# 3SAILab/two_stage_object_detection

Hardware: AMD Instinct MI355X
Metric: images/sec Faster R-CNN ResNet-50 @800x1333 (higher is better)
Workload: dtype f32 storage/accumulate; conv products as bf16x3 (3 exact bf16 pieces per operand, 6 bf16 MFMAs per product) in 0 of 43 conv layers, as fp16x2 (2 fp16 pieces of 2^e x per operand, 3 fp16 MFMAs per product; e follows the tensor's abs-max per forward: range words) in 43, f32 MFMA in the rest; 1 GPU; Full Faster R-CNN resnet50 inference forward, batch=1 per GPU, 3x800x1333, 80+1 classes, 3000->300 proposals; global_batch=1, parallelism=dp1, hip_graph=True, autotuned_tiles=True, steps_in_flight=4, tiles_tuned_on=this rank

## Files before the change

### include/tsod.h

```cpp
#ifndef TSOD_H
#define TSOD_H

#include <stddef.h>
#include <stdint.h>

#ifdef __cplusplus
extern "C" {
#endif

#define TSOD_VERSION 242

typedef void *tsod_stream_t;

typedef enum tsod_status {
    TSOD_OK = 0,
    TSOD_ERR_INVALID_ARG = -1,
    TSOD_ERR_UNSUPPORTED = -2,
    TSOD_ERR_ALIGNMENT = -3,
    TSOD_ERR_WORKSPACE = -4,
    TSOD_ERR_LAUNCH = -5
} tsod_status;

const char *tsod_status_str(int status);
int tsod_version(void);
int tsod_device_cu_count(void);

enum { TSOD_ACT_NONE = 0, TSOD_ACT_PRELU = 1, TSOD_ACT_RELU6 = 2, TSOD_ACT_RELU = 3 };
enum { TSOD_TILE_AUTO = 0, TSOD_TILE_128x128 = 1, TSOD_TILE_128x64 = 2, TSOD_TILE_64x64 = 3, TSOD_TILE_64x128 = 4,
       TSOD_TILE_128x128_W8 = 5, TSOD_TILE_128x64_W8 = 6, TSOD_TILE_256x128_W8 = 7, TSOD_TILE_64x64_S1 = 8,
       TSOD_TILE_128x64_W8_S1 = 9, TSOD_TILE_64x64_S1_K64 = 10, TSOD_TILE_128x64_W8_S1_K64 = 11,
       TSOD_TILE_64x64_W1_S1 = 12, TSOD_TILE_128x64_W2_S1 = 13, TSOD_TILE_128x64_S1 = 14, TSOD_TILE_64x128_S1 = 15,
       TSOD_TILE_128x128_S1 = 16,
       TSOD_TILE_D128x128 = 17, TSOD_TILE_D64x128 = 18, TSOD_TILE_D256x128 = 19,
       TSOD_TILE_D64x128_S2 = 20 ,
       TSOD_TILE_D128x256 = 21 ,
       TSOD_TILE_D128x128_K32 = 22 ,
       TSOD_TILE_D192x128 = 23 ,
       TSOD_TILE_D64x128_K64 = 24 ,
       TSOD_TILE_COUNT = 25 };
enum { TSOD_PREC_F32 = 0, TSOD_PREC_BF16X3 = 1, TSOD_PREC_FP16X2 = 2 };
#define TSOD_MAX_SEGMENTS 16

typedef struct tsod_conv2d_desc {
    int32_t N, H, W;
    int32_t in_pitch;
    int32_t n_seg;
    int32_t seg_off[TSOD_MAX_SEGMENTS];
    int32_t seg_len[TSOD_MAX_SEGMENTS];
    int32_t Cout;
    int32_t out_pitch;
    int32_t out_off;
    int32_t KH, KW;
    int32_t stride;
    int32_t pad_h, pad_w;
    int32_t OH, OW;
    int32_t act;
    float slope;
    int32_t res_pitch;
    int32_t res_off;
    int32_t tile;
    int32_t split_k;
    int32_t precision;
    int32_t c2, in2_pitch, in2_off, stride2, H2, W2;
    int32_t a_scale_exp, w_scale_exp;
    int32_t *range_flag;
    const uint32_t *amax_in, *amax_in2;
    uint32_t *amax_out;
} tsod_conv2d_desc;

#define TSOD_AMAX_WORDS 64
#define TSOD_AMAX_STRIDE 64
#define TSOD_AMAX_BYTES (TSOD_AMAX_WORDS * TSOD_AMAX_STRIDE)
int tsod_amax_reset(uint32_t *words, int32_t n_tensors, tsod_stream_t stream);
int tsod_absmax_f32(const float *x, int64_t n, uint32_t *amax_out, tsod_stream_t stream);

int tsod_host_mapped_pointer(void *host, void **device);
int tsod_word_publish_i32(const int32_t *src_device, int32_t *dst_mapped, tsod_stream_t stream);

int tsod_pack_conv_weight_f32(const float *w_oihw, int32_t Cout, int32_t Cin_src, int32_t KH, int32_t KW_src,
                              int32_t Cin, int32_t KW, float *w_packed, tsod_stream_t stream);

size_t tsod_conv_weight_bf16x3_bytes(int32_t Cout, int32_t K);
int tsod_pack_conv_weight_bf16x3(const float *w_packed , int32_t Cout, int32_t K, void *w_bf16x3,
                                 tsod_stream_t stream);
size_t tsod_conv_weight_fp16x2_bytes(int32_t Cout, int32_t K);
int tsod_pack_conv_weight_fp16x2(const float *w_packed , int32_t Cout, int32_t K, int32_t w_scale_exp,
                                 void *w_fp16x2, tsod_stream_t stream);

size_t tsod_conv2d_workspace_bytes(const tsod_conv2d_desc *d);
int tsod_conv2d_resolve(const tsod_conv2d_desc *d, int32_t *tile, int32_t *split_k);

int tsod_conv2d_f32(const tsod_conv2d_desc *d, const float *in, const float *w_packed,
                    const float *scale , const float *shift ,
                    const float *residual , float *out,
                    void *workspace, size_t workspace_bytes, tsod_stream_t stream);

int tsod_conv2d_dual_f32(const tsod_conv2d_desc *d, const float *in, const float *in2, const float *w_packed,
                         const float *scale, const float *shift, const float *residual, float *out,
                         void *workspace, size_t workspace_bytes, tsod_stream_t stream);

typedef struct tsod_bottleneck_desc {
    int32_t N, H, W;
    int32_t Cin, in_pitch;
    int32_t Cmid;
    int32_t Cout, out_pitch;
    float slope;
    int32_t w_exp[3];
    int32_t a_scale_exp;
    int32_t projection;
    int32_t *range_flag;
    const uint32_t *amax_in;
    uint32_t *amax_out;
} tsod_bottleneck_desc;
size_t tsod_bottleneck_wstream_bytes(int32_t Cin, int32_t Cout);
size_t tsod_bottleneck_proj_wstream_bytes(int32_t Cin, int32_t Cout);
int tsod_bottleneck_fp16x2(const tsod_bottleneck_desc *d, const float *x, const void *wstream, const float *bn, float *out,
                           tsod_stream_t stream);

#define TSOD_STEM_NCHW 0
#define TSOD_STEM_NHWC4 1
typedef struct tsod_stem_desc {
    int32_t N, H, W;
    int32_t in_layout;
    int32_t out_pitch;
    float slope;
    int32_t w_exp;
    int32_t *range_flag;
    uint32_t *amax_out;
} tsod_stem_desc;
size_t tsod_stem_wfrag_bytes(void);
int tsod_stem_fp16x2(const tsod_stem_desc *d, const float *x, const void *wfrag, const float *bn, float *out, tsod_stream_t stream);

int tsod_linear_f32(const float *in, int32_t M, int32_t K, int32_t in_pitch, const float *w ,
                    const float *bias , int32_t N, float *out, int32_t out_pitch,
                    void *workspace, size_t workspace_bytes, tsod_stream_t stream);
size_t tsod_linear_workspace_bytes(int32_t M, int32_t K, int32_t N);

int tsod_maxpool3x3s2_f32(const float *in, int32_t N, int32_t H, int32_t W, int32_t C, int32_t in_pitch,
                          float *out, int32_t out_pitch, tsod_stream_t stream);

int tsod_dwconv3x3_f32(const float *in, int32_t N, int32_t H, int32_t W, int32_t C, int32_t in_pitch, int32_t in_off,
                       const float *w, const float *scale, const float *shift, int32_t stride, int32_t relu,
                       float *out, int32_t out_pitch, int32_t out_off, tsod_stream_t stream);

int tsod_dwconv3x3_amax_f32(const float *in, int32_t N, int32_t H, int32_t W, int32_t C, int32_t in_pitch, int32_t in_off,
                            const float *w, const float *scale, const float *shift, int32_t stride, int32_t relu,
                            float *out, int32_t out_pitch, int32_t out_off, uint32_t *amax_out, tsod_stream_t stream);

int tsod_gconv3x3_f32(const float *in, int32_t N, int32_t H, int32_t W, int32_t C, int32_t in_pitch, int32_t groups,
                      const float *w, const float *scale, const float *shift, int32_t stride, int32_t act, float slope,
                      float *out, int32_t out_pitch, tsod_stream_t stream);

int tsod_gconv3x3_amax_f32(const float *in, int32_t N, int32_t H, int32_t W, int32_t C, int32_t in_pitch, int32_t groups,
                           const float *w, const float *scale, const float *shift, int32_t stride, int32_t act, float slope,
                           float *out, int32_t out_pitch, uint32_t *amax_out, tsod_stream_t stream);

int tsod_gconv1x1_pair_f32(const float *in, int64_t pixels, int32_t G, int32_t in_pitch, const float *w,
                           const float *bias, float *out, int32_t out_pitch, tsod_stream_t stream);

int tsod_gconv1x1_pair_amax_f32(const float *in, int64_t pixels, int32_t G, int32_t in_pitch, const float *w,
                                const float *bias, float *out, int32_t out_pitch, uint32_t *amax_out, tsod_stream_t stream);

int tsod_nchw_to_nhwc_f32(const float *in, int32_t N, int32_t C, int32_t H, int32_t W,
                          float *out, int32_t out_pitch, int32_t C_pad, tsod_stream_t stream);
int tsod_nchw_to_nhwc_amax_f32(const float *in, int32_t N, int32_t C, int32_t H, int32_t W,
                               float *out, int32_t out_pitch, int32_t C_pad, uint32_t *amax_out, tsod_stream_t stream);
int tsod_nhwc_to_nchw_f32(const float *in, int32_t N, int32_t C, int32_t H, int32_t W, int32_t in_pitch,
                          int32_t in_off, float *out, tsod_stream_t stream);

int tsod_rpn_decode_f32(const float *locs, int32_t loc_pitch, const float *scores, int32_t score_pitch,
                        const float *anchor_base , int32_t A, int32_t B, int32_t Hf, int32_t Wf,
                        int32_t feat_stride, float clamp_x, float clamp_y, float min_size,
                        float *boxes, float *fg, float *keys, float *anchors_out, tsod_stream_t stream);
// ... 333 lines not shown
```

### two_stage_object_detection_amd/_ffi.py

```python
from __future__ import annotations

import ctypes
import os
from ctypes import POINTER, Structure, byref, c_char_p, c_double, c_float, c_int, c_int32, c_int64, c_size_t, c_void_p
from typing import NamedTuple

import torch

_PKG_DIR = os.path.dirname(os.path.abspath(__file__))
LIB_PATH = os.environ.get("TSOD_LIB") or os.path.join(_PKG_DIR, "libtsod.so")

TSOD_MAX_SEGMENTS = 16
AMAX_WORDS, AMAX_STRIDE = 64, 64
AMAX_BYTES = AMAX_WORDS * AMAX_STRIDE
ACT_NONE, ACT_PRELU, ACT_RELU6, ACT_RELU = 0, 1, 2, 3
PREC_F32, PREC_BF16X3, PREC_FP16X2 = 0, 1, 2
PREC_NAMES = {0: "f32", 1: "bf16x3", 2: "fp16x2"}
TILE_AUTO, TILE_128x128, TILE_128x64, TILE_64x64, TILE_64x128 = 0, 1, 2, 3, 4


class Tile(NamedTuple):
    name: str
    rows: int
    precisions: tuple
# ... 37 lines not shown
TILE_NAMES = {TILE_AUTO: "auto", **{t: row.name for t, row in TILES.items()}}
TILE_IDS = tile_ids(PREC_F32)
DMA_TILE_IDS = tuple(t for t, row in TILES.items() if row.dma)
BF16X3_TILE_IDS = tile_ids(PREC_BF16X3)
FP16X2_TILE_IDS = tile_ids(PREC_FP16X2)

class TsodError(RuntimeError):
    pass


class ConvDesc(Structure):
    _fields_ = [
        ("N", c_int32), ("H", c_int32), ("W", c_int32),
        ("in_pitch", c_int32), ("n_seg", c_int32),
        ("seg_off", c_int32 * TSOD_MAX_SEGMENTS), ("seg_len", c_int32 * TSOD_MAX_SEGMENTS),
        ("Cout", c_int32), ("out_pitch", c_int32), ("out_off", c_int32),
        ("KH", c_int32), ("KW", c_int32), ("stride", c_int32), ("pad_h", c_int32), ("pad_w", c_int32),
        ("OH", c_int32), ("OW", c_int32), ("act", c_int32), ("slope", c_float),
        ("res_pitch", c_int32), ("res_off", c_int32), ("tile", c_int32), ("split_k", c_int32), ("precision", c_int32),
        ("c2", c_int32), ("in2_pitch", c_int32), ("in2_off", c_int32), ("stride2", c_int32), ("H2", c_int32), ("W2", c_int32),
        ("a_scale_exp", c_int32), ("w_scale_exp", c_int32), ("range_flag", c_void_p),
        ("amax_in", c_void_p), ("amax_in2", c_void_p), ("amax_out", c_void_p),
    ]


class BottleneckDesc(Structure):
    _fields_ = [
        ("N", c_int32), ("H", c_int32), ("W", c_int32), ("Cin", c_int32), ("in_pitch", c_int32), ("Cmid", c_int32),
        ("Cout", c_int32), ("out_pitch", c_int32), ("slope", c_float), ("w_exp", c_int32 * 3), ("a_scale_exp", c_int32),
        ("projection", c_int32), ("range_flag", c_void_p), ("amax_in", c_void_p), ("amax_out", c_void_p),
    ]


class StemDesc(Structure):
    _fields_ = [
        ("N", c_int32), ("H", c_int32), ("W", c_int32), ("in_layout", c_int32), ("out_pitch", c_int32), ("slope", c_float),
        ("w_exp", c_int32), ("range_flag", c_void_p), ("amax_out", c_void_p),
    ]


STEM_NCHW, STEM_NHWC4 = 0, 1

AUG_MEAN_PARTS = 256
AUG_BRIGHTNESS, AUG_CONTRAST, AUG_SATURATION, AUG_HUE, AUG_CONTRAST_FIRST, AUG_PERMUTE = 1, 2, 4, 8, 16, 32


class Photometric(Structure):
    _fields_ = [("flags", c_int32), ("brightness", c_float), ("contrast", c_float), ("saturation", c_float),
                ("hue", c_float), ("white", c_float), ("perm", c_int32 * 3)]


PW_MAX_SEGMENTS = 16


class PwSegs(Structure):
    _fields_ = [("n_seg", c_int32), ("off", c_int32 * PW_MAX_SEGMENTS), ("len", c_int32 * PW_MAX_SEGMENTS),
                ("real", c_int32 * PW_MAX_SEGMENTS), ("want", c_int32 * PW_MAX_SEGMENTS)]


ADAMW_CHUNK, ADAMW_MAX_GROUPS = 2048, 32
BN_ROWS_PER_WORKGROUP = 128


class AdamWGroup(Structure):
    _fields_ = [("decay", c_float), ("one_minus_beta1", c_float), ("beta2", c_float), ("one_minus_beta2", c_float),
                ("step_size", c_float), ("bias2_sqrt", c_float), ("eps", c_float), ("reserved", c_float)]


class GradNormResult(Structure):
    _fields_ = [("sum_sq", c_double), ("norm", c_float), ("coef", c_float)]


_SIGNATURES = {
    "tsod_status_str": (c_char_p, [c_int]),
    "tsod_version": (c_int, []),
    "tsod_device_cu_count": (c_int, []),
    "tsod_pack_conv_weight_f32": (c_int, [c_void_p, c_int32, c_int32, c_int32, c_int32, c_int32, c_int32, c_void_p, c_void_p]),
    "tsod_conv_weight_bf16x3_bytes": (c_size_t, [c_int32, c_int32]),
    "tsod_pack_conv_weight_bf16x3": (c_int, [c_void_p, c_int32, c_int32, c_void_p, c_void_p]),
    "tsod_conv_weight_fp16x2_bytes": (c_size_t, [c_int32, c_int32]),
    "tsod_pack_conv_weight_fp16x2": (c_int, [c_void_p, c_int32, c_int32, c_int32, c_void_p, c_void_p]),
    "tsod_conv2d_workspace_bytes": (c_size_t, [POINTER(ConvDesc)]),
    "tsod_conv2d_resolve": (c_int, [POINTER(ConvDesc), POINTER(c_int32), POINTER(c_int32)]),
    "tsod_conv2d_f32": (c_int, [POINTER(ConvDesc), c_void_p, c_void_p, c_void_p, c_void_p, c_void_p, c_void_p,
                                c_void_p, c_size_t, c_void_p]),
    "tsod_conv2d_dual_f32": (c_int, [POINTER(ConvDesc), c_void_p, c_void_p, c_void_p, c_void_p, c_void_p, c_void_p, c_void_p,
                                     c_void_p, c_size_t, c_void_p]),
    "tsod_bottleneck_wstream_bytes": (c_size_t, [c_int32, c_int32]),
    "tsod_bottleneck_proj_wstream_bytes": (c_size_t, [c_int32, c_int32]),
    "tsod_bottleneck_fp16x2": (c_int, [POINTER(BottleneckDesc), c_void_p, c_void_p, c_void_p, c_void_p, c_void_p]),
    "tsod_stem_wfrag_bytes": (c_size_t, []),
    "tsod_stem_fp16x2": (c_int, [POINTER(StemDesc), c_void_p, c_void_p, c_void_p, c_void_p, c_void_p]),
    "tsod_linear_f32": (c_int, [c_void_p, c_int32, c_int32, c_int32, c_void_p, c_void_p, c_int32, c_void_p, c_int32,
                                c_void_p, c_size_t, c_void_p]),
    "tsod_linear_workspace_bytes": (c_size_t, [c_int32, c_int32, c_int32]),
    "tsod_maxpool3x3s2_f32": (c_int, [c_void_p, c_int32, c_int32, c_int32, c_int32, c_int32, c_void_p, c_int32, c_void_p]),
    "tsod_dwconv3x3_f32": (c_int, [c_void_p, c_int32, c_int32, c_int32, c_int32, c_int32, c_int32, c_void_p, c_void_p,
                                   c_void_p, c_int32, c_int32, c_void_p, c_int32, c_int32, c_void_p]),
    "tsod_dwconv3x3_amax_f32": (c_int, [c_void_p, c_int32, c_int32, c_int32, c_int32, c_int32, c_int32, c_void_p, c_void_p,
                                        c_void_p, c_int32, c_int32, c_void_p, c_int32, c_int32, c_void_p, c_void_p]),
    "tsod_gconv3x3_amax_f32": (c_int, [c_void_p, c_int32, c_int32, c_int32, c_int32, c_int32, c_int32, c_void_p, c_void_p, c_void_p,
                                       c_int32, c_int32, c_float, c_void_p, c_int32, c_void_p, c_void_p]),
    "tsod_gconv1x1_pair_amax_f32": (c_int, [c_void_p, c_int64, c_int32, c_int32, c_void_p, c_void_p, c_void_p, c_int32, c_void_p, c_void_p]),
    "tsod_nchw_to_nhwc_amax_f32": (c_int, [c_void_p, c_int32, c_int32, c_int32, c_int32, c_void_p, c_int32, c_int32, c_void_p, c_void_p]),
    "tsod_absmax_f32": (c_int, [c_void_p, c_int64, c_void_p, c_void_p]),
    "tsod_amax_reset": (c_int, [c_void_p, c_int32, c_void_p]),
    "tsod_host_mapped_pointer": (c_int, [c_void_p, c_void_p]),
    "tsod_word_publish_i32": (c_int, [c_void_p, c_void_p, c_void_p]),
    "tsod_gconv3x3_f32": (c_int, [c_void_p, c_int32, c_int32, c_int32, c_int32, c_int32, c_int32, c_void_p, c_void_p, c_void_p,
                                  c_int32, c_int32, c_float, c_void_p, c_int32, c_void_p]),
    "tsod_gconv1x1_pair_f32": (c_int, [c_void_p, c_int64, c_int32, c_int32, c_void_p, c_void_p, c_void_p, c_int32, c_void_p]),
    "tsod_nchw_to_nhwc_f32": (c_int, [c_void_p, c_int32, c_int32, c_int32, c_int32, c_void_p, c_int32, c_int32, c_void_p]),
    "tsod_nhwc_to_nchw_f32": (c_int, [c_void_p, c_int32, c_int32, c_int32, c_int32, c_int32, c_int32, c_void_p, c_void_p]),
    "tsod_rpn_decode_f32": (c_int, [c_void_p, c_int32, c_void_p, c_int32, c_void_p, c_int32, c_int32, c_int32, c_int32,
                                    c_int32, c_float, c_float, c_float, c_void_p, c_void_p, c_void_p, c_void_p, c_void_p]),
    "tsod_proposal_decode_f32": (c_int, [c_void_p, c_void_p, c_void_p, c_int64, c_float, c_float, c_float, c_void_p,
                                         c_void_p, c_void_p]),
    "tsod_enumerate_anchors_f32": (c_int, [c_void_p, c_int32, c_int32, c_int32, c_int32, c_void_p, c_void_p]),
    "tsod_loc2bbox_f32": (c_int, [c_void_p, c_void_p, c_int64, c_void_p, c_void_p]),
    "tsod_bbox2loc_f32": (c_int, [c_void_p, c_void_p, c_int64, c_void_p, c_void_p]),
    "tsod_sort_topk_desc_f32": (c_int, [c_void_p, c_void_p, c_int32, c_int32, c_int32, c_void_p, c_void_p, c_void_p,
                                        c_void_p, c_void_p]),
    "tsod_sort_topk_workspace_bytes": (c_size_t, [c_int32, c_int32, c_int32]),
    "tsod_sort_topk_desc_ws_f32": (c_int, [c_void_p, c_void_p, c_int32, c_int32, c_int32, c_void_p, c_void_p, c_void_p,
                                           c_void_p, c_void_p, c_size_t, c_void_p]),
    "tsod_nms_workspace_bytes": (c_size_t, [c_int32, c_int32]),
    "tsod_nms_f32": (c_int, [c_void_p, c_void_p, c_int32, c_int32, c_float, c_int32, c_void_p, c_void_p, c_void_p,
                             c_void_p, c_void_p, c_size_t, c_void_p]),
    "tsod_bbox_iou_f32": (c_int, [c_void_p, c_int32, c_void_p, c_int32, c_float, c_void_p, c_void_p]),
    "tsod_roi_pool_f32": (c_int, [c_void_p, c_int32, c_int32, c_int32, c_int32, c_int32, c_void_p, c_int32, c_float,
                                  c_int32, c_int32, c_void_p, c_void_p]),
    "tsod_roi_pool_avg_f32": (c_int, [c_void_p, c_int32, c_int32, c_int32, c_int32, c_int32, c_void_p, c_void_p, c_int32,
                                      c_float, c_float, c_float, c_int32, c_int32, c_void_p, c_int32, c_void_p]),
    "tsod_roi_align_f32": (c_int, [c_void_p, c_int32, c_int32, c_int32, c_int32, c_int32, c_void_p, c_int32, c_float,
                                   c_int32, c_int32, c_int32, c_int32, c_void_p, c_void_p]),
    "tsod_roi_align_avg_f32": (c_int, [c_void_p, c_int32, c_int32, c_int32, c_int32, c_int32, c_void_p, c_void_p, c_int32,
                                       c_float, c_float, c_float, c_int32, c_int32, c_int32, c_int32, c_void_p, c_int32,
                                       c_void_p]),
    "tsod_detections_f32": (c_int, [c_void_p, c_int32, c_void_p, c_int32, c_void_p, c_int32, c_int32, c_void_p, c_void_p]),
    "tsod_resize_aa_taps": (c_int32, [c_int32, c_int32]),
    "tsod_resize_aa_tables_f32": (c_int, [c_int32, c_int32, c_void_p, c_void_p, c_void_p]),
    "tsod_resize_bilinear_aa_u8_f32": (c_int, [c_void_p, c_int32, c_int32, c_int32, c_int64, c_void_p, c_void_p, c_void_p,
                                               c_void_p, c_void_p, c_void_p, c_int32, c_int32, c_float, c_void_p, c_int64,
                                               c_int64, c_int64, c_int32, c_void_p]),
    "tsod_augment_gray_mean_partials": (c_int, [c_void_p, c_int32, c_int32, c_int64, POINTER(Photometric), c_void_p,
                                                c_void_p]),
    "tsod_augment_resize_u8_f32": (c_int, [c_void_p, c_int32, c_int32, c_int64, POINTER(Photometric), c_void_p, c_int32,
                                           c_void_p, c_void_p, c_void_p, c_void_p, c_void_p, c_void_p, c_int32, c_int32, c_void_p,
                                           c_int64, c_int64, c_int64, c_int32, c_void_p]),
    "tsod_resize_bilinear_aa_f32": (c_int, [c_void_p, c_int32, c_int32, c_int32, c_int64, c_int64, c_int64, c_void_p,
                                            c_void_p, c_void_p, c_void_p, c_void_p, c_void_p, c_int32, c_int32, c_void_p,
                                            c_int64, c_int64, c_int64, c_int32, c_void_p]),
    "tsod_augment_boxes_f32": (c_int, [c_void_p, c_void_p, c_int32, c_void_p, c_void_p, c_void_p, c_void_p, c_void_p,
                                       c_void_p]),
    "tsod_augment_color_host": (c_int, [c_void_p, c_int64, POINTER(Photometric), c_float, c_void_p]),
    "tsod_adamw_step_f32": (c_int, [c_void_p, c_int32, c_void_p, c_int64, c_void_p, c_int32, c_int32, c_void_p]),
    "tsod_adamw_step_host_f32": (c_int, [c_void_p, c_void_p, c_void_p, c_void_p, c_int64, POINTER(AdamWGroup), c_int32]),
    "tsod_grad_norm_workspace_bytes": (c_size_t, [c_int64]),
    "tsod_grad_norm_f32": (c_int, [c_void_p, c_int32, c_void_p, c_int64, c_float, c_void_p, c_void_p, c_size_t, c_void_p]),
    "tsod_adamw_step_clipped_f32": (c_int, [c_void_p, c_int32, c_void_p, c_int64, c_void_p, c_int32, c_int32, c_void_p,
                                            c_void_p]),
    "tsod_grad_scale_f32": (c_int, [c_void_p, c_int32, c_void_p, c_int64, c_void_p, c_void_p]),
    "tsod_grad_norm_host_f32": (c_int, [c_void_p, c_void_p, c_int32, c_float, POINTER(GradNormResult)]),
    "tsod_detection_keys_f32": (c_int, [c_void_p, c_int64, c_float, c_int32, c_void_p, c_void_p]),
    "tsod_gather_rows_f32": (c_int, [c_void_p, c_void_p, c_int32, c_int32, c_int32, c_int32, c_void_p, c_void_p]),
    "tsod_detection_nms_f32": (c_int, [c_void_p, c_void_p, c_int32, c_int32, c_float, c_int32, c_void_p, c_void_p, c_void_p,
# ... 225 lines not shown
```

### two_stage_object_detection_amd/csrc/conv_igemm_f32.hip

```cpp
#include "tsod_internal.h"
#include <array>
#include <limits.h>
#include <stdlib.h>

namespace {

typedef float f32x16 __attribute__((ext_vector_type(16)));
typedef __bf16 bf16x8 __attribute__((ext_vector_type(8)));
typedef _Float16 f16x8 __attribute__((ext_vector_type(8)));

constexpr int kPatchLD = 36;
constexpr int kChanTab = 512;

struct ConvParams {
    const float *in, *w, *scale, *shift, *res;
    float *out, *partial;
    int *tickets;
    unsigned part_bytes;
    int N, H, W, in_pitch;
    int n_seg, seg_off[TSOD_MAX_SEGMENTS], seg_end[TSOD_MAX_SEGMENTS];
    int Cin, Cout, out_pitch, out_off;
    int KH, KW, stride, pad_h, pad_w, OH, OW;
    int act;
    float slope;
// ... 1620 lines not shown
            s.split = 1; s.ksteps_per_split = ksteps; s.dp_tiles = 0; s.rem_tiles = s.tiles;
            s.ticket_bytes = kTicketBytes;
            s.ws_bytes = s.ticket_bytes + (size_t)grid * 2 * s.bm * s.bn * sizeof(float);
            const double step = (double)s.bm * s.bn / 4.0 * kTiles[tile].cost * (bk / 32.0) * 0.55;
            const double fixed = 3000.0 + (double)s.bm * s.bn / 8.0;
            s.cost = (double)q * step + fixed * (1.0 + (double)q / ksteps) + 2500.0 + 2.0 * s.bm * s.bn * 4.0 / 60.0;
            return s;
        }
        s.cost = 1e300;
        s.split = 1; s.ksteps_per_split = ksteps; s.dp_tiles = s.tiles; s.rem_tiles = 0; s.grid = s.tiles; s.ws_bytes = 0; s.ticket_bytes = 0;
        return s;
    }
    int split = 1, dp = s.tiles;
    if (mode > 1) {
        split = mode < ksteps ? mode : ksteps;
        dp = 0;
    } else if (mode == -1) {
        const int full = s.tiles / slots * slots;
        const int rem = s.tiles - full;
        if (rem > 0) {
            split = slots / rem;
            if (split > ksteps / 2) split = ksteps / 2;
            if (split < 1) split = 1;
            if (split > 1) dp = full;
        }
    }
    int kps = (ksteps + split - 1) / split;
    split = (ksteps + kps - 1) / kps;
    if (split <= 1 || (size_t)(s.tiles - dp) * sizeof(int) > kTicketBytes) {
        split = 1; dp = s.tiles; kps = ksteps;
    }
    s.split = split; s.ksteps_per_split = kps; s.dp_tiles = dp; s.rem_tiles = s.tiles - dp;
    s.grid = dp + s.rem_tiles * split;
    if ((dp == s.tiles || dp == 0) && s.tiles_n >= 2 && s.grid >= 16) {
        const double wbytes = (double)d->Cout * K * (d->precision ? 6.0 : 4.0);
        const double abytes = (double)d->N * d->H * d->W * desc_cin(d) * 4.0 + (d->c2 > 0 ? (double)M * d->c2 * 4.0 : 0.0);
        const double g = s.tiles_n < 8 ? s.tiles_n : 8;
        const int force = xcd_map_override();
        s.nmajor = force >= 0 ? force : (8.0 * wbytes * (1.0 - 1.0 / g) > abytes * (g - 1.0) * 1.25 ? 1 : 0);
    }
    s.ticket_bytes = s.rem_tiles > 0 ? kTicketBytes : 0;
    s.ws_bytes = s.ticket_bytes + (size_t)s.rem_tiles * split * s.bm * s.bn * sizeof(float);

    const double step = (double)s.bm * s.bn / 4.0 * kTiles[tile].cost * (bk / 32.0) * (d->precision ? 0.55 : 1.0);
    const double fixed = 3000.0 + (double)s.bm * s.bn / 8.0;
    const int cus = cu_count();
    double c = (double)tsod_cdiv(dp, cus) * (ksteps * step + fixed);
    if (s.rem_tiles > 0)
        c += (double)tsod_cdiv((int64_t)s.rem_tiles * split, cus) * (kps * step + fixed) + 2500.0 +
             (double)split * s.bm * s.bn * 4.0 / 60.0;
    s.cost = c;
    return s;
}

Sched resolve(const tsod_conv2d_desc *d) {
    Sched best;
    best.cost = 1e300;
    for (int t = 1; t < TSOD_TILE_COUNT; ++t) {
        if (d->tile != TSOD_TILE_AUTO && d->tile != t) continue;
        if (!kTiles[t].launch[d->precision]) continue;
        if (!tile_ok_for(d, t)) continue;
        if (d->split_k != 0) {
            const Sched s = make_sched(d, t, d->split_k);
            if (s.cost < best.cost) best = s;
            continue;
        }
        const int K = desc_k(d);
        const int ksteps = (K + kTiles[t].bk - 1) / kTiles[t].bk;
        for (int mode : {1, -1, 2, 4, 8, 16, -2}) {
            if (mode > 1 && ksteps / mode < 2) continue;
            if (mode == -2 && !kTiles[t].dma) continue;
            const Sched s = make_sched(d, t, mode);
            if (s.cost < best.cost) best = s;
        }
    }
    return best;
}

uint64_t weight_image_bytes(int prec, int Cout, int K) {
    const uint64_t groups = (uint64_t)Cout * ((K + 7) / 8);
    return prec == TSOD_PREC_BF16X3 ? groups * 48 : prec == TSOD_PREC_FP16X2 ? groups * 32 : (uint64_t)Cout * K * sizeof(float);
}

}

extern "C" int tsod_conv2d_resolve(const tsod_conv2d_desc *d, int32_t *tile, int32_t *split_k) {
    const int rc = validate(d);
    if (rc != TSOD_OK) return rc;
    TSOD_REQUIRE(tile && split_k, TSOD_ERR_INVALID_ARG);
    const Sched s = resolve(d);
    TSOD_REQUIRE(s.cost < 1e299, TSOD_ERR_UNSUPPORTED);
    *tile = s.tile;
    *split_k = s.sk_q > 0 ? -2 : (s.rem_tiles == 0 ? 1 : (s.dp_tiles == 0 ? s.split : -1));
    return TSOD_OK;
}

extern "C" size_t tsod_conv2d_workspace_bytes(const tsod_conv2d_desc *d) {
    if (validate(d) != TSOD_OK) return 0;
    const Sched s = resolve(d);
    return s.cost < 1e299 ? s.ws_bytes : 0;
}

extern "C" int tsod_conv2d_f32(const tsod_conv2d_desc *d, const float *in, const float *w_packed, const float *scale,
                               const float *shift, const float *residual, float *out, void *workspace,
                               size_t workspace_bytes, tsod_stream_t stream) {
    if (d != nullptr && d->c2 != 0) return TSOD_ERR_INVALID_ARG;
    return tsod_conv2d_dual_f32(d, in, nullptr, w_packed, scale, shift, residual, out, workspace, workspace_bytes, stream);
}

extern "C" int tsod_conv2d_dual_f32(const tsod_conv2d_desc *d, const float *in, const float *in2, const float *w_packed,
                                    const float *scale, const float *shift, const float *residual, float *out,
                                    void *workspace, size_t workspace_bytes, tsod_stream_t stream) {
    const int rc = validate(d);
    if (rc != TSOD_OK) return rc;
    TSOD_REQUIRE(in && w_packed && out, TSOD_ERR_INVALID_ARG);
    TSOD_REQUIRE((d->c2 > 0) == (in2 != nullptr) && (!in2 || tsod_aligned16(in2)), TSOD_ERR_INVALID_ARG);
    TSOD_REQUIRE(tsod_aligned16(in) && tsod_aligned16(w_packed), TSOD_ERR_ALIGNMENT);
    if (residual) TSOD_REQUIRE(d->res_off >= 0 && d->res_pitch >= d->res_off + d->Cout, TSOD_ERR_INVALID_ARG);

    ConvParams p;
    p.in = in; p.w = w_packed; p.scale = scale; p.shift = shift; p.res = residual; p.out = out;
    p.N = d->N; p.H = d->H; p.W = d->W; p.in_pitch = d->in_pitch;
    p.n_seg = d->n_seg;
    int cum = 0;
    for (int s = 0; s < TSOD_MAX_SEGMENTS; ++s) {
        p.seg_off[s] = s < d->n_seg ? d->seg_off[s] : 0;
        if (s < d->n_seg) cum += d->seg_len[s];
        p.seg_end[s] = cum;
    }
    p.Cin = cum; p.Cout = d->Cout; p.out_pitch = d->out_pitch; p.out_off = d->out_off;
    p.KH = d->KH; p.KW = d->KW; p.stride = d->stride; p.pad_h = d->pad_h; p.pad_w = d->pad_w;
    p.OH = d->OH; p.OW = d->OW; p.act = d->act; p.slope = d->slope;
    p.res_pitch = d->res_pitch; p.res_off = d->res_off;
    p.M = d->N * d->OH * d->OW;
    p.K1 = d->KH * d->KW * p.Cin;
    p.K = desc_k(d);
    p.in2 = in2; p.c2 = d->c2 > 0 ? d->c2 : 0; p.in2_pitch = d->in2_pitch; p.in2_off = d->in2_off;
    p.stride2 = d->stride2; p.H2 = d->H2; p.W2 = d->W2;
    {
        const uint64_t in2_bytes = in2 ? (uint64_t)d->N * d->H2 * d->W2 * d->in2_pitch * sizeof(float) : 0;
        TSOD_REQUIRE(in2_bytes < 0xFFFFFFF0ull, TSOD_ERR_UNSUPPORTED);
        p.in2_bytes = (unsigned)in2_bytes;
        const uint64_t in_bytes = (uint64_t)d->N * d->H * d->W * d->in_pitch * sizeof(float);
        const uint64_t w_bytes = weight_image_bytes(d->precision, d->Cout, p.K);
        const uint64_t out_bytes = (uint64_t)p.M * d->out_pitch * sizeof(float);
        const uint64_t res_bytes = residual ? (uint64_t)p.M * d->res_pitch * sizeof(float) : 0;
        TSOD_REQUIRE(in_bytes < 0xFFFFFFF0ull && w_bytes < 0xFFFFFFF0ull && out_bytes < 0xFFFFFFF0ull &&
                         res_bytes < 0xFFFFFFF0ull && p.K < (1 << 21),
                     TSOD_ERR_UNSUPPORTED);
        p.in_bytes = (unsigned)in_bytes;
        p.w_bytes = (unsigned)w_bytes;
        p.out_bytes = (unsigned)out_bytes;
        p.res_bytes = (unsigned)res_bytes;
        p.neg_slope = d->act == TSOD_ACT_NONE ? 1.f : (d->act == TSOD_ACT_PRELU ? d->slope : 0.f);
        p.act_hi = d->act == TSOD_ACT_RELU6 ? 6.f : __builtin_huge_valf();
        p.vec_epilogue = ((d->Cout | d->out_pitch | d->out_off) & 3) == 0 && tsod_aligned16(out) &&
                         (!residual || (((d->res_pitch | d->res_off) & 3) == 0 && tsod_aligned16(residual))) &&
                         (!scale || tsod_aligned16(scale)) && (!shift || tsod_aligned16(shift));
        p.inv_cin = 1.0f / (float)p.Cin;
        p.inv_kw = 1.0f / (float)d->KW;
    }
    const Sched sc = resolve(d);
    TSOD_REQUIRE(sc.cost < 1e299, TSOD_ERR_UNSUPPORTED);
    p.uniform_tap = (d->n_seg == 1 && p.Cin % kTiles[sc.tile].bk == 0) ? 1 : 0;
    p.chan_tab = (kTiles[sc.tile].dma && dma_chan_case(d)) ? 1 : 0;
    p.pointwise_tab = (!p.uniform_tap && !kTiles[sc.tile].dma && d->KH == 1 && d->KW == 1 && d->pad_h == 0 && d->pad_w == 0 && d->stride == 1 &&
                       p.c2 == 0 && p.K <= 4 * kChanTab) ? 1 : 0;
    TSOD_REQUIRE(p.c2 == 0 || (p.uniform_tap && p.K1 % kTiles[sc.tile].bk == 0 && p.c2 % kTiles[sc.tile].bk == 0), TSOD_ERR_UNSUPPORTED);
    p.ksteps = (p.K + kTiles[sc.tile].bk - 1) / kTiles[sc.tile].bk;
    p.tiles_m = sc.tiles_m; p.tiles_n = sc.tiles_n;
    p.dp_tiles = sc.dp_tiles; p.split = sc.split; p.ksteps_per_split = sc.ksteps_per_split; p.sk_q = sc.sk_q;
    p.nmajor = sc.nmajor;
    const int cblk = kTiles[sc.tile].bk > 32 ? kTiles[sc.tile].bk : 32;
    p.cmajor = (kTiles[sc.tile].dma && d->KH * d->KW > 1 && p.Cin % cblk == 0) ? 1 : 0;
    p.ci_wrap = p.cmajor ? cblk : p.Cin;
    if (sc.rem_tiles > 0)
        TSOD_REQUIRE(workspace != nullptr && workspace_bytes >= sc.ws_bytes && tsod_aligned16(workspace), TSOD_ERR_WORKSPACE);
    p.tickets = static_cast<int *>(workspace);
    p.partial = reinterpret_cast<float *>(static_cast<char *>(workspace) + sc.ticket_bytes);
    p.part_bytes = (unsigned)(sc.ws_bytes - sc.ticket_bytes);
    TSOD_REQUIRE(sc.ws_bytes < 0xFFFFFFF0ull, TSOD_ERR_UNSUPPORTED);
    hipStream_t s = tsod_stream(stream);
    p.a_scale = 1.f; p.acc_scale = 1.f; p.range_flag = nullptr;
    p.amax_in = nullptr; p.amax_in2 = nullptr; p.w_scale_exp = 0;
    p.amax_out = d->amax_out;
    TSOD_REQUIRE((reinterpret_cast<uintptr_t>(d->amax_out) & 63u) == 0 && (reinterpret_cast<uintptr_t>(d->amax_in) & 63u) == 0 &&
                     (reinterpret_cast<uintptr_t>(d->amax_in2) & 63u) == 0, TSOD_ERR_ALIGNMENT);
    if (d->precision == TSOD_PREC_FP16X2) {
        p.range_flag = d->range_flag;
        p.amax_in = d->amax_in;
        p.amax_in2 = (d->amax_in != nullptr && p.c2 > 0) ? d->amax_in2 : nullptr;
        p.w_scale_exp = d->w_scale_exp;
        p.a_scale = ldexpf(1.f, d->a_scale_exp);
        p.acc_scale = ldexpf(1.f, -(d->a_scale_exp + d->w_scale_exp));
    }
    kTiles[sc.tile].launch[d->precision](p, sc.grid, s);
    return tsod_launch_status();
}

extern "C" size_t tsod_linear_workspace_bytes(int32_t M, int32_t K, int32_t N) {
    if (M <= 0 || K <= 0 || N <= 0) return 0;
    tsod_conv2d_desc d = {};
    d.N = 1; d.H = 1; d.W = M; d.in_pitch = K; d.n_seg = 1; d.seg_off[0] = 0; d.seg_len[0] = K;
    d.Cout = N; d.out_pitch = N; d.KH = 1; d.KW = 1; d.stride = 1; d.OH = 1; d.OW = M;
    return tsod_conv2d_workspace_bytes(&d);
}

extern "C" int tsod_linear_f32(const float *in, int32_t M, int32_t K, int32_t in_pitch, const float *w,
                               const float *bias, int32_t N, float *out, int32_t out_pitch, void *workspace,
                               size_t workspace_bytes, tsod_stream_t stream) {
    TSOD_REQUIRE(M > 0 && K > 0 && N > 0, TSOD_ERR_INVALID_ARG);
    TSOD_REQUIRE((K & 3) == 0, TSOD_ERR_ALIGNMENT);
    tsod_conv2d_desc d = {};
    d.N = 1; d.H = 1; d.W = M; d.in_pitch = in_pitch; d.n_seg = 1; d.seg_off[0] = 0; d.seg_len[0] = K;
    d.Cout = N; d.out_pitch = out_pitch; d.KH = 1; d.KW = 1; d.stride = 1; d.OH = 1; d.OW = M;
    d.act = TSOD_ACT_NONE;
    return tsod_conv2d_f32(&d, in, w, nullptr, bias, nullptr, out, workspace, workspace_bytes, stream);
}

extern "C" int tsod_pack_conv_weight_f32(const float *w_oihw, int32_t Cout, int32_t Cin_src, int32_t KH, int32_t KW_src,
                                         int32_t Cin, int32_t KW, float *w_packed, tsod_stream_t stream) {
    TSOD_REQUIRE(w_oihw && w_packed, TSOD_ERR_INVALID_ARG);
    TSOD_REQUIRE(Cout > 0 && Cin_src > 0 && KH > 0 && KW_src > 0 && Cin >= Cin_src && KW >= KW_src, TSOD_ERR_INVALID_ARG);
    const long total = (long)Cout * KH * KW * Cin;
    const int blocks = (int)(tsod_cdiv(total, 256) < 4096 ? tsod_cdiv(total, 256) : 4096);
    hipLaunchKernelGGL(pack_weight_kernel, dim3(blocks), dim3(256), 0, tsod_stream(stream), w_oihw, Cout, Cin_src, KH,
                       KW_src, Cin, KW, w_packed);
    return tsod_launch_status();
}

extern "C" size_t tsod_conv_weight_bf16x3_bytes(int32_t Cout, int32_t K) {
    if (Cout <= 0 || K <= 0) return 0;
    return weight_image_bytes(TSOD_PREC_BF16X3, Cout, K);
}

extern "C" int tsod_pack_conv_weight_bf16x3(const float *w_packed, int32_t Cout, int32_t K, void *w_bf16x3, tsod_stream_t stream) {
    TSOD_REQUIRE(w_packed && w_bf16x3, TSOD_ERR_INVALID_ARG);
    TSOD_REQUIRE(Cout > 0 && K > 0, TSOD_ERR_INVALID_ARG);
    TSOD_REQUIRE(tsod_aligned16(w_bf16x3), TSOD_ERR_ALIGNMENT);
    const long total = (long)Cout * ((K + 7) / 8);
    const int blocks = (int)(tsod_cdiv(total, 256) < 4096 ? tsod_cdiv(total, 256) : 4096);
    hipLaunchKernelGGL(pack_weight_bf16x3_kernel, dim3(blocks), dim3(256), 0, tsod_stream(stream), w_packed, Cout, K,
                       static_cast<unsigned *>(w_bf16x3));
    return tsod_launch_status();
}

extern "C" size_t tsod_conv_weight_fp16x2_bytes(int32_t Cout, int32_t K) {
// ... 28 lines not shown
```

### two_stage_object_detection_amd/csrc/tsod_internal.h

```cpp
#pragma once
#include <hip/hip_runtime.h>
#include <stdint.h>
#include "../../include/tsod.h"

#define TSOD_WAVE 64

static inline hipStream_t tsod_stream(tsod_stream_t s) { return reinterpret_cast<hipStream_t>(s); }

static inline int tsod_launch_status() {
    return hipGetLastError() == hipSuccess ? TSOD_OK : TSOD_ERR_LAUNCH;
}

static inline bool tsod_aligned16(const void *p) { return (reinterpret_cast<uintptr_t>(p) & 15u) == 0; }

static inline int64_t tsod_cdiv(int64_t a, int64_t b) { return (a + b - 1) / b; }

static inline size_t tsod_align_up(size_t v, size_t a) { return (v + a - 1) / a * a; }

#define TSOD_REQUIRE(cond, code) \
    do {                         \
        if (!(cond)) return (code); \
    } while (0)


#ifdef __HIPCC__
#define TSOD_AMAX_STRIDE_WORDS (TSOD_AMAX_STRIDE / 4)
__device__ __forceinline__ float tsod_wave_max(float v) {
#pragma unroll
    for (int o = 32; o > 0; o >>= 1) v = fmaxf(v, __shfl_xor(v, o));
    return v;
}
__device__ __forceinline__ float tsod_block_max(float v, float *scr, int tid) {
    v = tsod_wave_max(v);
    __syncthreads();
    if ((tid & 63) == 0) scr[tid >> 6] = v;
    __syncthreads();
    return fmaxf(fmaxf(scr[0], scr[1]), fmaxf(scr[2], scr[3]));
}
__device__ __forceinline__ void tsod_amax_commit(unsigned *amax, float mx, float *smem, int tid, int nthreads) {
    mx = tsod_wave_max(mx);
    __syncthreads();
    if ((tid & 63) == 0) smem[tid >> 6] = mx;
    __syncthreads();
    if (tid == 0) {
        for (int w = 1; w < nthreads / 64; ++w) mx = fmaxf(mx, smem[w]);
        atomicMax(amax + (blockIdx.x % TSOD_AMAX_WORDS) * TSOD_AMAX_STRIDE_WORDS, __float_as_uint(mx));
    }
}
__device__ __forceinline__ unsigned tsod_amax_reduce_bits(unsigned mine) {
#pragma unroll
    for (int o = 32; o > 0; o >>= 1) { const unsigned other = (unsigned)__shfl_xor((int)mine, o); mine = other > mine ? other : mine; }
    return (unsigned)__builtin_amdgcn_readfirstlane((int)mine);
}
static_assert(TSOD_AMAX_WORDS == 64, "one word per lane of a wave");
struct tsod_box { float x1, y1, x2, y2; };
__device__ __forceinline__ tsod_box tsod_decode_box(float ax1, float ay1, float ax2, float ay2,
                                                    float dx, float dy, float dw, float dh) {
    const float w = ax2 - ax1;
    const float h = ay2 - ay1;
    const float cx = ax1 + 0.5f * w;
    const float cy = ay1 + 0.5f * h;
    const float ncx = dx * w + cx;
    const float ncy = dy * h + cy;
    const float nw = expf(dw) * w;
    const float nh = expf(dh) * h;
    tsod_box o;
    o.x1 = ncx - 0.5f * nw;
    o.y1 = ncy - 0.5f * nh;
    o.x2 = ncx + 0.5f * nw;
    o.y2 = ncy + 0.5f * nh;
    return o;
}
__device__ __forceinline__ bool tsod_argmax_takes(float v, int c, float best, int bi) {
    if (c == 0x7fffffff) return false;
    if (bi == 0x7fffffff) return true;
    const bool vn = v != v, bn = best != best;
    if (vn || bn) return vn && (!bn || c < bi);
    return v > best || (v == best && c < bi);
}
__device__ __forceinline__ void tsod_wave_argmax(const float *s, int n_class, int lane, float &best, int &bi) {
    best = -INFINITY;
    bi = 0x7fffffff;
    for (int c = lane; c < n_class; c += 64) {
        const float v = s[c];
        if (tsod_argmax_takes(v, c, best, bi)) { best = v; bi = c; }
    }
    for (int off = 32; off > 0; off >>= 1) {
        const float ov = __shfl_xor(best, off);
        const int oi = __shfl_xor(bi, off);
        if (tsod_argmax_takes(ov, oi, best, bi)) { best = ov; bi = oi; }
    }
}
__device__ __forceinline__ float4 tsod_roi_to_map(float4 rr, float img_h, float img_w, int Hf, int Wf) {
    return make_float4(rr.x / img_w * (float)Wf, rr.y / img_h * (float)Hf, rr.z / img_w * (float)Wf, rr.w / img_h * (float)Hf);
}
struct tsod_pool_geom {
    int b, sw, sh, rw, rh;
};
__device__ __forceinline__ tsod_pool_geom tsod_roi_pool_geom(float bidx, float x1, float y1, float x2, float y2, float scale) {
    tsod_pool_geom g;
    g.b = (int)bidx;
    g.sw = (int)roundf(x1 * scale);
    g.sh = (int)roundf(y1 * scale);
    const int ew = (int)roundf(x2 * scale);
    const int eh = (int)roundf(y2 * scale);
    g.rw = max(ew - g.sw + 1, 1);
// ... 73 lines not shown
```

Baseline: 1202 images/s.

## Add panel kernel for fp16x2 1x1 expand convs keeping activations resident in LDS

Adds a specialised implicit-GEMM kernel for stride-1 1x1 fp16x2 convolutions with small Cin (64-128) and Cout at least twice Cin. Each workgroup splits a 64-row activation panel into hi/lo fp16 planes once in LDS, then sweeps over the output-channel blocks with double-buffered weight registers and a fused scale/shift/residual/activation/amax epilogue. The aim is to avoid re-loading and re-splitting the activation tile for every output-channel tile, at the cost of a new code path, an alignment requirement, and a fixed grid split that may give poor occupancy on some shapes.

```diff
diff --git a/include/tsod.h b/include/tsod.h
--- a/include/tsod.h
+++ b/include/tsod.h
@@ -89,6 +89,7 @@
 
 size_t tsod_conv2d_workspace_bytes(const tsod_conv2d_desc *d);
 int tsod_conv2d_resolve(const tsod_conv2d_desc *d, int32_t *tile, int32_t *split_k);
+int tsod_conv2d_uses_panel(const tsod_conv2d_desc *d);
 
 int tsod_conv2d_f32(const tsod_conv2d_desc *d, const float *in, const float *w_packed,
                     const float *scale , const float *shift ,
diff --git a/two_stage_object_detection_amd/_ffi.py b/two_stage_object_detection_amd/_ffi.py
--- a/two_stage_object_detection_amd/_ffi.py
+++ b/two_stage_object_detection_amd/_ffi.py
@@ -143,6 +143,7 @@
     "tsod_pack_conv_weight_fp16x2": (c_int, [c_void_p, c_int32, c_int32, c_int32, c_void_p, c_void_p]),
     "tsod_conv2d_workspace_bytes": (c_size_t, [POINTER(ConvDesc)]),
     "tsod_conv2d_resolve": (c_int, [POINTER(ConvDesc), POINTER(c_int32), POINTER(c_int32)]),
+    "tsod_conv2d_uses_panel": (c_int, [POINTER(ConvDesc)]),
     "tsod_conv2d_f32": (c_int, [POINTER(ConvDesc), c_void_p, c_void_p, c_void_p, c_void_p, c_void_p, c_void_p,
                                 c_void_p, c_size_t, c_void_p]),
     "tsod_conv2d_dual_f32": (c_int, [POINTER(ConvDesc), c_void_p, c_void_p, c_void_p, c_void_p, c_void_p, c_void_p, c_void_p,
diff --git a/two_stage_object_detection_amd/csrc/conv_igemm_f32.hip b/two_stage_object_detection_amd/csrc/conv_igemm_f32.hip
--- a/two_stage_object_detection_amd/csrc/conv_igemm_f32.hip
+++ b/two_stage_object_detection_amd/csrc/conv_igemm_f32.hip
@@ -1726,6 +1726,29 @@
     return prec == TSOD_PREC_BF16X3 ? groups * 48 : prec == TSOD_PREC_FP16X2 ? groups * 32 : (uint64_t)Cout * K * sizeof(float);
 }
 
+int panel_rows(const tsod_conv2d_desc *d, const Sched &sc) {
+    if (d->precision != TSOD_PREC_FP16X2 || sc.tile != TSOD_TILE_64x128_S1 || sc.rem_tiles != 0 || sc.sk_q != 0) return 0;
+    if (d->KH != 1 || d->KW != 1 || d->stride != 1 || d->pad_h != 0 || d->pad_w != 0 || d->n_seg != 1 || d->c2 > 0) return 0;
+    if (d->OH != d->H || d->OW != d->W) return 0;
+    const int Cin = d->seg_len[0];
+    if (Cin % 32 != 0 || Cin < 64 || Cin > 128 || d->Cout % 128 != 0 || d->Cout < 2 * Cin) return 0;
+    if ((d->in_pitch | d->seg_off[0] | d->out_pitch | d->out_off | d->res_pitch | d->res_off) & 3) return 0;
+    return 64;
+}
+
+int panel_nsplit(int64_t M, int Cout, int rows) {
+    const int64_t panels = tsod_cdiv(M, rows);
+    int n = 1;
+    while (n < 4 && Cout % (256 * n) == 0 && panels * n * 2 <= 2 * cu_count()) n *= 2;
+    return n;
+}
+
+}
+
+extern "C" int tsod_conv2d_uses_panel(const tsod_conv2d_desc *d) {
+    if (validate(d) != TSOD_OK) return 0;
+    const Sched s = resolve(d);
+    return s.cost < 1e299 ? panel_rows(d, s) : 0;
 }
 
 extern "C" int tsod_conv2d_resolve(const tsod_conv2d_desc *d, int32_t *tile, int32_t *split_k) {
@@ -1806,7 +1829,21 @@
     }
     const Sched sc = resolve(d);
     TSOD_REQUIRE(sc.cost < 1e299, TSOD_ERR_UNSUPPORTED);
-    p.uniform_tap = (d->n_seg == 1 && p.Cin % kTiles[sc.tile].bk == 0) ? 1 : 0;
+    if (const int rows = panel_rows(d, sc); rows > 0 && p.vec_epilogue) {
+        TSOD_REQUIRE((reinterpret_cast<uintptr_t>(d->amax_out) & 63u) == 0 && (reinterpret_cast<uintptr_t>(d->amax_in) & 63u) == 0, TSOD_ERR_ALIGNMENT);
+        tsod_panel_params q;
+        q.in = in; q.scale = scale; q.shift = shift; q.res = residual; q.w = w_packed; q.out = out;
+        q.M = p.M; q.Cin = p.Cin; q.Cout = d->Cout;
+        q.in_pitch = d->in_pitch; q.in_off = d->seg_off[0]; q.out_pitch = d->out_pitch; q.out_off = d->out_off;
+        q.res_pitch = d->res_pitch; q.res_off = d->res_off;
+        q.in_bytes = p.in_bytes; q.w_bytes = p.w_bytes; q.out_bytes = p.out_bytes; q.res_bytes = p.res_bytes;
+        q.neg_slope = p.neg_slope; q.act_hi = p.act_hi;
+        q.a_scale_exp = d->a_scale_exp; q.w_scale_exp = d->w_scale_exp;
+        q.amax_in = d->amax_in; q.amax_out = d->amax_out; q.range_flag = d->range_flag;
+        q.nsplit = panel_nsplit(p.M, d->Cout, rows);
+        return tsod_conv_panel_launch(q, tsod_stream(stream));
+    }
+    p.uniform_tap =(d->n_seg == 1 && p.Cin % kTiles[sc.tile].bk == 0) ? 1 : 0;
     p.chan_tab = (kTiles[sc.tile].dma && dma_chan_case(d)) ? 1 : 0;
     p.pointwise_tab = (!p.uniform_tap && !kTiles[sc.tile].dma && d->KH == 1 && d->KW == 1 && d->pad_h == 0 && d->pad_w == 0 && d->stride == 1 &&
                        p.c2 == 0 && p.K <= 4 * kChanTab) ? 1 : 0;
diff --git a/two_stage_object_detection_amd/csrc/conv_panel.hip b/two_stage_object_detection_amd/csrc/conv_panel.hip
--- /dev/null
+++ b/two_stage_object_detection_amd/csrc/conv_panel.hip
@@ -0,0 +1,214 @@
+#include "tsod_internal.h"
+
+namespace {
+
+typedef float f32x16 __attribute__((ext_vector_type(16)));
+typedef unsigned int u32x4 __attribute__((ext_vector_type(4)));
+
+constexpr unsigned kOOB = 0xFFFFFFF0u;
+constexpr int P_PITCH = 144, P_BYTES = 32 * P_PITCH;
+
+__device__ __forceinline__ float4 bload4(__amdgpu_buffer_rsrc_t r, unsigned off) {
+    const u32x4 v = __builtin_amdgcn_raw_buffer_load_b128(r, off, 0, 0);
+    return make_float4(__uint_as_float(v.x), __uint_as_float(v.y), __uint_as_float(v.z), __uint_as_float(v.w));
+}
+__device__ __forceinline__ float act1(float v, float neg_slope, float hi) {
+    return fminf(fmaxf(v, 0.f) + neg_slope * fminf(v, 0.f), hi);
+}
+
+template <int PB, int NCH>
+__global__ void __launch_bounds__(256, 2) conv_igemm_kernel_panel(const tsod_panel_params p) {
+    constexpr int ROWS = 32 * PB, PITCH = NCH * 32 + 16, PLANE = ROWS * PITCH;
+    constexpr int PATCH_OFF = 2 * PLANE, SCR_OFF = PATCH_OFF + 4 * P_BYTES, LDS_BYTES = SCR_OFF + 64;
+    constexpr int NX = ROWS * NCH * 4 / 256;
+    static_assert(PB * NCH == 16 && NX == 8 && 2 * LDS_BYTES <= 160 * 1024, "panel geometry; two workgroups per CU");
+    __shared__ __align__(16) unsigned char lds[LDS_BYTES];
+    const int tid = threadIdx.x, lane = tid & 63, wave = tid >> 6;
+    const int j = lane & 31, hh = lane >> 5;
+    const int nch = p.Cin >> 4;
+    const int panel = (int)blockIdx.x / p.nsplit, part = (int)blockIdx.x - panel * p.nsplit;
+    const int m0 = panel * ROWS;
+    const int nq = p.Cout / (128 * p.nsplit);
+    const int cb0 = part * (4 * nq) + wave;
+    float *scr = reinterpret_cast<float *>(lds + SCR_OFF);
+
+    const __amdgpu_buffer_rsrc_t rs_x = __builtin_amdgcn_make_buffer_rsrc((void *)p.in, (short)0, (int)p.in_bytes, 0x00020000);
+    const __amdgpu_buffer_rsrc_t rs_w = __builtin_amdgcn_make_buffer_rsrc((void *)p.w, (short)0, (int)p.w_bytes, 0x00020000);
+    const __amdgpu_buffer_rsrc_t rs_o = __builtin_amdgcn_make_buffer_rsrc((void *)p.out, (short)0, (int)p.out_bytes, 0x00020000);
+    const __amdgpu_buffer_rsrc_t rs_r = __builtin_amdgcn_make_buffer_rsrc((void *)(p.res ? p.res : p.out), (short)0,
+                                                                           (int)(p.res ? p.res_bytes : 0u), 0x00020000);
+    const bool has_res = p.res != nullptr;
+
+    unsigned range_bits = 0;
+    if (p.amax_in != nullptr) range_bits = p.amax_in[lane * TSOD_AMAX_STRIDE_WORDS];
+    float4 xr[NX];
+    int xdst[NX];
+    {
+        const int upr = p.Cin >> 2, n_units = ROWS * upr;
+#pragma unroll
+        for (int i = 0; i < NX; ++i) {
+            const int u = tid + 256 * i, row = u / upr, q4 = u - row * upr;
+            const int m = m0 + row;
+            const bool in_panel = u < n_units;
+            xdst[i] = in_panel ? row * PITCH + q4 * 8 : -1;
+            xr[i] = bload4(rs_x, (in_panel && m < p.M) ? ((unsigned)m * (unsigned)p.in_pitch + (unsigned)(p.in_off + q4 * 4)) * 4u : kOOB);
+        }
+    }
+    const int lrow = lane >> 3, lpiece = lane & 7;
+    const unsigned wrow_bytes = (unsigned)p.Cin * 4u;
+    const unsigned wlane = (unsigned)lrow * wrow_bytes + (unsigned)lpiece * 16u;
+    u32x4 wreg[NCH / 2][4];
+    auto w_load = [&](int cp, unsigned base) {
+        const unsigned o = (base != kOOB && 2 * cp < nch) ? base + (unsigned)cp * 128u : kOOB;
+#pragma unroll
+        for (int t = 0; t < 4; ++t) wreg[cp][t] = __builtin_amdgcn_raw_buffer_load_b128(rs_w, o != kOOB ? o + (unsigned)(8 * t) * wrow_bytes : kOOB, 0, 0);
+    };
+    {
+        const unsigned base = (unsigned)(cb0 * 32) * wrow_bytes + wlane;
+#pragma unroll
+        for (int cp = 0; cp < NCH / 2; ++cp) w_load(cp, base);
+    }
+    const int pi = 16 * ((j >> 2) & 1) + 4 * (j >> 3) + (j & 3);
+    int wst[2], wrd[2][2];
+#pragma unroll
+    for (int t = 0; t < 2; ++t) wst[t] = (8 * t + lrow) * 128 + ((lpiece ^ (((8 * t + lrow) >> 1) & 7)) << 4);
+#pragma unroll
+    for (int s = 0; s < 2; ++s)
+#pragma unroll
+        for (int hl = 0; hl < 2; ++hl) wrd[s][hl] = pi * 128 + (((4 * s + 2 * hh + hl) ^ ((pi >> 1) & 7)) << 4);
+    int e_x = p.a_scale_exp;
+    if (p.amax_in != nullptr) e_x = tsod_fp16x2_exp_from_bits(tsod_amax_reduce_bits(range_bits));
+    e_x = __builtin_amdgcn_readfirstlane(e_x);
+    const float a_scale = __uint_as_float((unsigned)(127 + e_x) << 23);
+    const float acc_scale = __uint_as_float((unsigned)(127 - e_x - p.w_scale_exp) << 23);
+
+    const int ep_px = lane >> 3, ep_q = lane & 7;
+    unsigned opix[PB][4], rpix[PB][4];
+#pragma unroll
+    for (int b = 0; b < PB; ++b)
+#pragma unroll
+        for (int i = 0; i < 4; ++i) {
+            const int m = m0 + b * 32 + ep_px + 8 * i;
+            const bool ok = m < p.M;
+            opix[b][i] = ok ? ((unsigned)m * (unsigned)p.out_pitch + (unsigned)(p.out_off + ep_q * 4)) * 4u : kOOB;
+            rpix[b][i] = (ok && has_res) ? ((unsigned)m * (unsigned)p.res_pitch + (unsigned)(p.res_off + ep_q * 4)) * 4u : kOOB;
+        }
+    float4 res[PB][4], sc4, sh4;
+    auto side_load = [&](int cb) {
+        const unsigned chb = (unsigned)(cb * 32) * 4u;
+        if (has_res) {
+#pragma unroll
+            for (int b = 0; b < PB; ++b)
+#pragma unroll
+                for (int i = 0; i < 4; ++i) res[b][i] = bload4(rs_r, rpix[b][i] != kOOB ? rpix[b][i] + chb : kOOB);
+        }
+        sc4 = p.scale ? *reinterpret_cast<const float4 *>(p.scale + cb * 32 + ep_q * 4) : make_float4(1.f, 1.f, 1.f, 1.f);
+        sh4 = p.shift ? *reinterpret_cast<const float4 *>(p.shift + cb * 32 + ep_q * 4) : make_float4(0.f, 0.f, 0.f, 0.f);
+    };
+#pragma unroll
+    for (int b = 0; b < PB; ++b)
+#pragma unroll
+        for (int i = 0; i < 4; ++i) res[b][i] = make_float4(0.f, 0.f, 0.f, 0.f);
+
+#pragma unroll
+    for (int i = 0; i < NX; ++i) {
+        if (xdst[i] >= 0) {
+            unsigned h0, l0, h1, l1;
+            tsod_split2_pair(xr[i].x, xr[i].y, a_scale, h0, l0);
+            tsod_split2_pair(xr[i].z, xr[i].w, a_scale, h1, l1);
+            *reinterpret_cast<uint2 *>(lds + xdst[i]) = make_uint2(h0, h1);
+            *reinterpret_cast<uint2 *>(lds + PLANE + xdst[i]) = make_uint2(l0, l1);
+        }
+    }
+    side_load(cb0);
+    __syncthreads();
+
+    const int xfa = j * PITCH + hh * 16;
+    unsigned char *patch = lds + PATCH_OFF + wave * P_BYTES;
+    struct AFrag { u32x4 h, l; };
+    AFrag af[2][PB];
+    auto a_frags = [&](int c, AFrag (&f)[PB]) {
+#pragma unroll
+        for (int b = 0; b < PB; ++b) {
+            f[b].h = *reinterpret_cast<const u32x4 *>(lds + xfa + b * 32 * PITCH + c * 32);
+            f[b].l = *reinterpret_cast<const u32x4 *>(lds + xfa + b * 32 * PITCH + c * 32 + PLANE);
+        }
+    };
+    auto w_stage = [&](int cp) {
+#pragma unroll
+        for (int t = 0; t < 4; ++t) *reinterpret_cast<u32x4 *>(patch + wst[t & 1] + (t >> 1) * 2048) = wreg[cp][t];
+    };
+    float amax = 0.f;
+    bool bad = false;
+    for (int q = 0; q < nq; ++q) {
+        const int cb = cb0 + 4 * q;
+        const unsigned wnext = q + 1 < nq ? (unsigned)((cb + 4) * 32) * wrow_bytes + wlane : kOOB;
+        f32x16 acc[PB];
+#pragma unroll
+        for (int b = 0; b < PB; ++b)
+#pragma unroll
+            for (int e = 0; e < 16; ++e) acc[b][e] = 0.f;
+        a_frags(0, af[0]);
+        w_stage(0);
+#pragma unroll
+        for (int cp = 0; cp < NCH / 2; ++cp) {
+            if (2 * cp < nch) {
+                u32x4 wh[2], wl[2];
+#pragma unroll
+                for (int s = 0; s < 2; ++s) {
+                    wh[s] = *reinterpret_cast<const u32x4 *>(patch + wrd[s][0]);
+                    wl[s] = *reinterpret_cast<const u32x4 *>(patch + wrd[s][1]);
+                }
+                if (cp + 1 < NCH / 2) w_stage(cp + 1);
+#pragma unroll
+                for (int s = 0; s < 2; ++s) {
+                    const int c = 2 * cp + s;
+                    if (c + 1 < NCH) a_frags(c + 1, af[(c + 1) & 1]);
+#pragma unroll
+                    for (int b = 0; b < PB; ++b) tsod_mfma3(acc[b], wh[s], wl[s], af[c & 1][b].h, af[c & 1][b].l);
+                }
+            }
+            w_load(cp, wnext);
+        }
+        const unsigned chb = (unsigned)(cb * 32) * 4u;
+#pragma unroll
+        for (int b = 0; b < PB; ++b) {
+#pragma unroll
+            for (int v = 0; v < 4; ++v) {
+                const float a0 = acc[b][4 * v] * acc_scale, a1 = acc[b][4 * v + 1] * acc_scale;
+                const float a2 = acc[b][4 * v + 2] * acc_scale, a3 = acc[b][4 * v + 3] * acc_scale;
+                bad = bad || !(fabsf(a0) <= 3.4028234664e38f) || !(fabsf(a1) <= 3.4028234664e38f) || !(fabsf(a2) <= 3.4028234664e38f) ||
+                      !(fabsf(a3) <= 3.4028234664e38f);
+                *reinterpret_cast<float4 *>(patch + j * P_PITCH + (16 * hh + 4 * v) * 4) = make_float4(a0, a1, a2, a3);
+            }
+            asm volatile("s_waitcnt lgkmcnt(0)" ::: "memory");
+            float4 t[4];
+#pragma unroll
+            for (int i = 0; i < 4; ++i) t[i] = *reinterpret_cast<const float4 *>(patch + (ep_px + 8 * i) * P_PITCH + ep_q * 16);
+            asm volatile("s_waitcnt lgkmcnt(0)" ::: "memory");
+#pragma unroll
+            for (int i = 0; i < 4; ++i) {
+                const float o0 = act1(t[i].x * sc4.x + sh4.x + res[b][i].x, p.neg_slope, p.act_hi);
+                const float o1 = act1(t[i].y * sc4.y + sh4.y + res[b][i].y, p.neg_slope, p.act_hi);
+                const float o2 = act1(t[i].z * sc4.z + sh4.z + res[b][i].z, p.neg_slope, p.act_hi);
+                const float o3 = act1(t[i].w * sc4.w + sh4.w + res[b][i].w, p.neg_slope, p.act_hi);
+                const float m4 = fmaxf(fmaxf(fabsf(o0), fabsf(o1)), fmaxf(fabsf(o2), fabsf(o3)));
+                amax = fmaxf(amax, opix[b][i] != kOOB ? m4 : 0.f);
+                u32x4 o;
+                o.x = __float_as_uint(o0); o.y = __float_as_uint(o1); o.z = __float_as_uint(o2); o.w = __float_as_uint(o3);
+                __builtin_amdgcn_raw_buffer_store_b128(o, rs_o, opix[b][i] != kOOB ? opix[b][i] + chb : kOOB, 0, 0);
+            }
+        }
+        if (q + 1 < nq) side_load(cb + 4);
+    }
+    if (p.range_flag != nullptr && __any(bad) && lane == 0) atomicOr(p.range_flag, 1);
+    if (p.amax_out != nullptr) tsod_amax_commit(p.amax_out, amax, scr, tid, 256);
+}
+
+}
+
+int tsod_conv_panel_launch(const tsod_panel_params &p, hipStream_t s) {
+    const int grid = (int)tsod_cdiv(p.M, 64) * p.nsplit;
+    hipLaunchKernelGGL((conv_igemm_kernel_panel<2, 8>), dim3((unsigned)grid), dim3(256), 0, s, p);
+    return tsod_launch_status();
+}
diff --git a/two_stage_object_detection_amd/csrc/tsod_internal.h b/two_stage_object_detection_amd/csrc/tsod_internal.h
--- a/two_stage_object_detection_amd/csrc/tsod_internal.h
+++ b/two_stage_object_detection_amd/csrc/tsod_internal.h
@@ -22,6 +22,21 @@
         if (!(cond)) return (code); \
     } while (0)
 
+struct tsod_panel_params {
+    const float *in, *scale, *shift, *res;
+    const void *w;
+    float *out;
+    int M, Cin, Cout;
+    int in_pitch, in_off, out_pitch, out_off, res_pitch, res_off;
+    unsigned in_bytes, w_bytes, out_bytes, res_bytes;
+    float neg_slope, act_hi;
+    int a_scale_exp, w_scale_exp;
+    const unsigned *amax_in;
+    unsigned *amax_out;
+    int *range_flag;
+    int nsplit;
+};
+int tsod_conv_panel_launch(const tsod_panel_params &p, hipStream_t s);
 
 #ifdef __HIPCC__
 #define TSOD_AMAX_STRIDE_WORDS (TSOD_AMAX_STRIDE / 4)
```

Measured after the change: 1205 images/s, median of 2. About the same (+0.2%).
